# yohanshin/MultiviewHMR

Measured on AMD Instinct MI355X. Metric: Mvoxel*views/s (64^3 grid, 256ch, 4 views) fwd; max-abs vs ref, higher is better.
Workload: dtype f32

## Files before the change

### multiviewhmr_amd/csrc/brick_common.h

```cpp
#pragma once
#include <type_traits>
#include "device_common.h"

namespace mvhmr {

constexpr int kBZ = 32;
constexpr int kBX = 4;
constexpr int kMaxChunks = 5;
constexpr int brick_chunks_per_wave(int nt) { return nt >= 1024 ? kMaxChunks : 2 * kMaxChunks; }
constexpr int brick_view_slots(int v) { return v <= 2 ? 2 : v <= 4 ? 4 : 8; }

struct BrickTiles { int hx, hy, hz, share; bool split_x, split_y, split_z; };
__host__ __device__ inline BrickTiles brick_tiles(int nbx, int nby, int nbz)
{
    BrickTiles t;
    t.split_z = nbz >= 2;
    t.split_x = t.split_z ? nbx > nby : true;
    t.split_y = t.split_z ? !t.split_x : true;
    t.hx = t.split_x ? (nbx + 1) / 2 : nbx; t.hy = t.split_y ? (nby + 1) / 2 : nby; t.hz = t.split_z ? (nbz + 1) / 2 : nbz;
    t.share = t.hx * t.hy * t.hz;
    return t;
}

constexpr int kAbsentSlot = 64;
constexpr float kAbsentSample = -3.4028234663852886e38f;
constexpr int kZeroSlots = 128;
constexpr int kZeroBytes = kZeroSlots * 16;

__device__ __forceinline__ void lds_barrier()
{
    asm volatile("s_waitcnt lgkmcnt(0)\n\ts_barrier" ::: "memory");
}

__device__ __forceinline__ void bare_barrier()
{
    asm volatile("s_barrier" ::: "memory");
}
// ... 162 lines not shown
```

### multiviewhmr_amd/csrc/capi.hip

```cpp
#include "mvhmr_unproject.h"

#include <hip/hip_runtime.h>
#include <stdarg.h>
#include <stdio.h>

#include <mutex>
#include <unordered_map>

#include "device_common.h"
#include "kernels.h"

using namespace mvhmr;

namespace mvhmr {
unsigned long long dynamic_lds_cache_key(int device, const void *kernel)
{
    return (unsigned long long)reinterpret_cast<uintptr_t>(kernel) ^ ((unsigned long long)(unsigned)device << 56) ^ (unsigned long long)(device & 0xff);
}

hipError_t allow_dynamic_lds(const void *kernel, size_t bytes)
{
    static std::mutex mu;
    static std::unordered_map<unsigned long long, size_t> granted;
    int dev = 0;
    hipError_t e = hipGetDevice(&dev);
    if (e != hipSuccess) return e;
    const unsigned long long key = dynamic_lds_cache_key(dev, kernel);
    std::lock_guard<std::mutex> lock(mu);
    auto it = granted.find(key);
    if (it != granted.end() && it->second >= bytes) return hipSuccess;
    e = hipFuncSetAttribute(kernel, hipFuncAttributeMaxDynamicSharedMemorySize, (int)bytes);
    if (e == hipSuccess) granted[key] = bytes;
    return e;
}
}

namespace {

thread_local char g_err[512] = "";

int fail(int status, const char *fmt, ...)
{
    va_list ap;
    va_start(ap, fmt);
    vsnprintf(g_err, sizeof(g_err), fmt, ap);
    va_end(ap);
    return status;
}
// ... 88 lines not shown
bool gateable_layout(const mvhmr_unproject_desc *d, const Problem &p)
{
    return d->feat_layout == MVHMR_LAYOUT_BVCHW || (d->feat_layout == MVHMR_LAYOUT_QUAD && quad_to_channels_last_supported(p));
}
bool geometry_gated(const mvhmr_unproject_desc *d, const Problem &p)
{
    return d->variant == MVHMR_VARIANT_AUTO && gateable_layout(d, p) && brick_fwd_preferred(p);
}
bool geometry_gated_bwd(const mvhmr_unproject_desc *d, const Problem &p)
{
    return d->variant == MVHMR_VARIANT_AUTO && gateable_layout(d, p) && brick_bwd_supported(p);
}
constexpr size_t kGateBytes = 256;
size_t conv_bytes(const Problem &p) { const size_t a = featT_bytes(p), b = brick_workspace_bytes(p); return a > b ? a : b; }

int arm_gate(Problem &p, unsigned char *at, const float *proj, const Coords &coords, const GateGeom &g, hipStream_t s)
{
    int *count = reinterpret_cast<int *>(at);
    hipError_t e = hipMemsetAsync(count, 0, sizeof(int), s);
    if (e != hipSuccess) return fail(MVHMR_ERR_LAUNCH, "geometry gate clear: %s", hipGetErrorString(e));
    e = launch_brick_gate(proj, coords, count, g, p, s);
    if (e != hipSuccess) return fail(MVHMR_ERR_LAUNCH, "geometry gate: %s", hipGetErrorString(e));
    p.gate_count = count;
    p.gate_limit = brick_count(p, g) / 8;
    return MVHMR_OK;
}

int check_ws(void *ws, size_t have, size_t need)
{
    if (need == 0) return MVHMR_OK;
    if (!ws) return fail(MVHMR_ERR_WORKSPACE, "workspace is null but %zu bytes are required", need);
    if (have < need) return fail(MVHMR_ERR_WORKSPACE, "workspace has %zu bytes, %zu are required", have, need);
    if (reinterpret_cast<uintptr_t>(ws) % kAlign) return fail(MVHMR_ERR_WORKSPACE, "workspace must be %zu-byte aligned", kAlign);
    return MVHMR_OK;
}

Coords coords_from_tensor(const float *coords, const Problem &p)
{
    Coords c{};
// ... 416 lines not shown
}
int clear_gradient(void *acc, const Problem &p, size_t elem, hipStream_t s)
{
    return launched(hipMemsetAsync(acc, 0, (size_t)p.B * p.V * p.H * p.W * p.C4 * elem, s), "gradient clear");
}
int query_variant(const mvhmr_unproject_desc *desc, const VolumeSource &v, const float *proj, void *hip_stream)
{
    Problem p;
    if (check_desc(desc, &p) != MVHMR_OK) return -1;
    const int variant = pick_variant(desc, p);
    if (variant_conflict(desc, p, variant) != MVHMR_OK) return -1;
    if (desc->variant != MVHMR_VARIANT_AUTO || !brick_fwd_preferred(p)) return variant;
    Coords coords;
    if (!proj || make_coords(v, p, &coords) != MVHMR_OK) { fail(MVHMR_ERR_INVALID_ARGUMENT, v.cuboid ? "null pointer" : "proj / coords must be non-null"); return -1; }
    hipStream_t s = static_cast<hipStream_t>(hip_stream);
    int *count = nullptr, host = 0;
    if (hipMalloc(&count, sizeof(int)) != hipSuccess) { fail(MVHMR_ERR_LAUNCH, "query: allocation failed"); return -1; }
    hipError_t e = hipMemsetAsync(count, 0, sizeof(int), s);
    const GateGeom g = brick_fwd_gate_geom(p);
    if (e == hipSuccess) e = launch_brick_gate(proj, coords, count, g, p, s);
    if (e == hipSuccess) e = hipMemcpyAsync(&host, count, sizeof(int), hipMemcpyDeviceToHost, s);
    if (e == hipSuccess) e = hipStreamSynchronize(s);
    (void)hipFree(count);
    if (e != hipSuccess) { fail(MVHMR_ERR_LAUNCH, "query: %s", hipGetErrorString(e)); return -1; }
    return host <= brick_count(p, g) / 8 ? MVHMR_VARIANT_BRICK : MVHMR_VARIANT_GATHER;
}

int run_forward(const mvhmr_unproject_desc *desc, const VolumeSource &v, const void *features, const float *proj, const Views &views, void *out,
                void *workspace, size_t workspace_bytes, void *hip_stream, const SharedIndex *shared = nullptr, const LensArgs *lens = nullptr)
{
    Problem p0;
    Coords coords;
    int rc = open_call(desc, v, &p0, &coords);
    if (rc != MVHMR_OK) return rc;
    if (!features || !proj || !out) return fail(MVHMR_ERR_INVALID_ARGUMENT, "features / proj / out must be non-null");
    if ((rc = views_refused(desc, views)) != MVHMR_OK) return rc;
    if (shared && (rc = shared_refused(desc, *shared)) != MVHMR_OK) return rc;
    if (lens && (rc = lens_refused(desc, *lens)) != MVHMR_OK) return rc;
    if (lens) p0.lens = lens->lens;
    hipStream_t s = static_cast<hipStream_t>(hip_stream);
// ... 1097 lines not shown
```

### multiviewhmr_amd/csrc/device_common.h

```cpp
#pragma once
#include <hip/hip_runtime.h>
#include <hip/hip_fp16.h>
#include <stdint.h>
#include "gate.h"

namespace mvhmr {

__device__ __forceinline__ bool gated_off(const Gate &g)
{
    if (!g.count) return false;
    const bool brick = __builtin_nontemporal_load(g.count) <= g.limit;
    return brick != (g.wants_brick != 0);
}


__device__ __forceinline__ void cuboid_offset(const Coords &cs, int b, long long n, float &dx, float &dy, float &dz)
{
    const int k = (int)(n % cs.Z), j = (int)((n / cs.Z) % cs.Y), i = (int)(n / ((long long)cs.Y * cs.Z));
    const float *ce = cs.center + b * 3;
    const float gx = __fadd_rn(cs.px, __fmul_rn(cs.sx, (float)i));
    const float gy = __fadd_rn(cs.py, __fmul_rn(cs.sy, (float)j));
    const float gz = __fadd_rn(cs.pz, __fmul_rn(cs.sz, (float)k));
    dx = __fsub_rn(gx, ce[0]); dy = __fsub_rn(gy, ce[1]); dz = __fsub_rn(gz, ce[2]);
}

__device__ __forceinline__ void voxel_xyz(const Coords &cs, int b, long long N, long long n, float &x, float &y, float &z)
{
// ... 554 lines not shown
```

### multiviewhmr_amd/csrc/gate.h

```cpp
#pragma once

namespace mvhmr {

struct Gate {
    const int *count;
    int limit;
    int wants_brick;
};

struct Coords {
    const float *ptr;
    const float *rot;
    const float *center;
    float px, py, pz;
    float sx, sy, sz;
    int Y, Z;
};

}
```

### multiviewhmr_amd/csrc/kernels.h

```cpp
#pragma once
#include <hip/hip_runtime.h>
#include <stddef.h>
#include <stdint.h>
#include "gate.h"

namespace mvhmr {

struct Problem {
    int B, V, C, H, W;
    int X, Y, Z;
    long long N;
    int C4;
    int method;
    int feat_f16, out_f16;
    int out_bf16 = 0;
    int feat_log2e = 0;
    const int *gate_count = nullptr;
    int gate_limit = 0;
    const int *view_count = nullptr;
    const float *view_weights = nullptr;
    int masked = 0;
    int visible = 0;
    const float *confidence = nullptr;
    int conf = 0;
    float *conf_stream = nullptr;
    const int *feature_index = nullptr;
    int volumes = 0;
    const float *lens = nullptr;
};

inline Gate make_gate(const Problem &p, bool wants_brick) { return Gate{p.gate_count, p.gate_limit, wants_brick ? 1 : 0}; }


hipError_t allow_dynamic_lds(const void *kernel, size_t bytes);
unsigned long long dynamic_lds_cache_key(int device, const void *kernel);

hipError_t launch_to_channels_last(const void *src, void *dst, const Problem &p, hipStream_t s);
hipError_t launch_grad_to_planar(const float *srcT, void *dst, const Problem &p, hipStream_t s);
bool quad_to_channels_last_supported(const Problem &p);
hipError_t launch_quad_to_channels_last(const void *srcK, void *dst, const Problem &p, hipStream_t s);
hipError_t launch_grad_cast(const float *srcT, void *dst, const Problem &p, hipStream_t s);

hipError_t launch_fwd_gather(const void *featT, const float *proj, const Coords &coords, void *out,
                             const Problem &p, hipStream_t s);
hipError_t launch_bwd_gather(const void *grad_out, const void *featT, const float *proj, const Coords &coords,
                             float *gradT, const Problem &p, hipStream_t s);

// ... 25 lines not shown
hipError_t launch_bwd_plane(const void *featK, const void *grad_out, const float *proj, const Coords &coords, void *grad_features,
                            void *table, const Problem &p, hipStream_t s);

struct GateGeom {
    int bx, by, bz;
    int view_group;
    int column_major;
    int parity_rows;
    int cap_slots;
    int max_chunks;
};
GateGeom brick_fwd_gate_geom(const Problem &p);
GateGeom brick_bwd_gate_geom(const Problem &p);
hipError_t launch_brick_gate(const float *proj, const Coords &coords, int *count, const GateGeom &g, const Problem &p, hipStream_t s);
int brick_count(const Problem &p, const GateGeom &g);

hipError_t launch_bwd_brick(const void *featK, const void *grad_out, const float *proj, const Coords &coords, float *gradK,
                            const Problem &p, hipStream_t s);
hipError_t launch_quad_grad_to_planar(const float *gradK, void *dst, const Problem &p, hipStream_t s);

bool conv1x1_quad_supported(int Cin, int Cout, int H, int W);
bool conv1x1_planar_supported(int Cin, int Cout, int HW);
bool conv1x1_wgrad_supported(int Cin, int Cout, int HW);
hipError_t launch_conv1x1_wgrad(const float *gy, const float *x, float *dW, float *db, int BV, int Cin, int Cout, int HW, hipStream_t s);
size_t conv1x1_wgrad_det_workspace_bytes(int BV, int Cin, int Cout, int HW);
hipError_t launch_conv1x1_wgrad_det(const float *gy, const float *x, float *dW, float *db, void *ws, int BV, int Cin, int Cout, int HW, hipStream_t s);
constexpr int kConv1x1MaxMaps = 65535;
hipError_t launch_conv1x1_planar(const float *x, const float *w, const float *bias, float *dst, int BV, int Cin, int Cout, int HW, hipStream_t s);
hipError_t launch_conv1x1_quad(const float *x, const float *w, const float *bias, void *dst, int BV, int Cin, int Cout, int H, int W,
                               hipStream_t s);
// ... 81 lines not shown
```

### multiviewhmr_amd/csrc/unproject_brick_fwd.hip

```cpp
#include "brick_fwd_ws.h"

namespace mvhmr {

template <typename TF>
__global__ void __launch_bounds__(256)
k_to_quad_planar_t(const TF *__restrict__ src, float4 *__restrict__ dst, int C, int H, int W, float scale, Gate gate)
{
    if (gated_off(gate)) return;
    __shared__ float tile[4][32][33];
    const long long bv = blockIdx.z;
    const int q = blockIdx.y;
    const int tiles_x = (W + 31) >> 5;
    const int x0 = (blockIdx.x % tiles_x) << 5, y0 = (blockIdx.x / tiles_x) << 5;
    const int tx = threadIdx.x & 31, ty = threadIdx.x >> 5;
    const TF *s = src + (bv * C + q * 4) * (long long)H * W;
    const int nc = C - q * 4 < 4 ? C - q * 4 : 4;
#pragma unroll
    for (int c = 0; c < 4; ++c)
#pragma unroll
        for (int i = 0; i < 4; ++i) {
            const int y = y0 + ty + 8 * i, x = x0 + tx;
            if (y < H && x < W) tile[c][ty + 8 * i][tx] = c < nc ? to_f32<TF>(s[(long long)c * H * W + (long long)y * W + x]) * scale : 0.f;
        }
    __syncthreads();
// ... 148 lines not shown
    const int nt = brick_fwd_grouped(p) ? 1024 : fwd_threads(p.V);
    GateGeom g;
    g.bx = kBX * brick_fwd_nvox(p); g.by = nt / 128; g.bz = kBZ; g.column_major = 1;
    g.parity_rows = kFwdLay == 1 ? 1 : 0;
    g.view_group = brick_fwd_grouped(p) ? 4 : 0;
    g.cap_slots = fwd_cap2(fwd_lds_slots());
    g.max_chunks = brick_fwd_grouped(p) ? 4 * (nt / 64) : brick_chunks_per_wave(nt) * (nt / 64);
    return g;
}

int brick_count(const Problem &p, const GateGeom &g)
{
    return ((p.X + g.bx - 1) / g.bx) * ((p.Y + g.by - 1) / g.by) * ((p.Z + g.bz - 1) / g.bz) * p.B;
}

__global__ void __launch_bounds__(256)
k_brick_gate(const float *__restrict__ proj, const Coords coords, int *__restrict__ count, int V, int H, int W, int X,
             int Y, int Z, GateGeom g, int nbx, int nby, int nbz, int total)
{
    const int i = blockIdx.x * 256 + threadIdx.x;
    if (i >= total) return;
    const int bps = nbx * nby * nbz;
    const int b = i / bps, r = i % bps;
    const int kz = r % nbz, ky = (r / nbz) % nby, kx = r / (nbz * nby);
    const long long N = (long long)X * Y * Z;
    int used = 0, chunks_all = 0, max_stride = 0, used_max = 0, chunks_max = 0;
    for (int v = 0; v < V; ++v) {
        if (g.view_group && v % g.view_group == 0) { used = 0; chunks_all = 0; }
        const float *P = proj + ((long long)b * V + v) * 12;
        float xmin = 1e30f, xmax = -1e30f, ymin = 1e30f, ymax = -1e30f;
        bool front = true;
        for (int c = 0; c < 8; ++c) {
            int vx = kx * g.bx + ((c & 1) ? g.bx - 1 : 0), vy = ky * g.by + ((c & 2) ? g.by - 1 : 0), vz = kz * g.bz + ((c & 4) ? g.bz - 1 : 0);
            vx = vx < X ? vx : X - 1; vy = vy < Y ? vy : Y - 1; vz = vz < Z ? vz : Z - 1;
            float Xp[3];
            voxel_xyz(coords, b, N, ((long long)vx * Y + vy) * Z + vz, Xp[0], Xp[1], Xp[2]);
            const float a = P[0] * Xp[0] + P[1] * Xp[1] + P[2] * Xp[2] + P[3];
            const float bb = P[4] * Xp[0] + P[5] * Xp[1] + P[6] * Xp[2] + P[7];
            const float z = P[8] * Xp[0] + P[9] * Xp[1] + P[10] * Xp[2] + P[11];
            if (!(z > 0.f)) { front = false; continue; }
            const float ix = (a / z) / (float)H * (float)(W - 1), iy = (bb / z) / (float)W * (float)(H - 1);
            xmin = fminf(xmin, ix); xmax = fmaxf(xmax, ix); ymin = fminf(ymin, iy); ymax = fmaxf(ymax, iy);
        }
        if (!front || xmax < xmin) continue;
        const float x0 = fmaxf(floorf(xmin), -1.f), x1 = fminf(floorf(xmax), (float)(W - 1));
        const float y0 = fmaxf(floorf(ymin), -1.f), y1 = fminf(floorf(ymax), (float)(H - 1));
        if (x1 < x0 || y1 < y0) continue;
        const int bw = (int)(x1 - x0) + 2, bh = (int)(y1 - y0) + 2;
        int stride = (g.column_major ? bh : bw) | 1;
        const int lines = g.column_major ? bw : bh;
        if (g.parity_rows) {
            const int y0e = (int)y0 & ~1;
            stride = 2 * (((int)y1 + 3 - y0e) >> 1);
        }
        const int chunks = (stride * lines + 63) >> 6;
        used += chunks << 6;
        chunks_all += chunks;
        max_stride = stride > max_stride ? stride : max_stride;
        used_max = used > used_max ? used : used_max;
        chunks_max = chunks_all > chunks_max ? chunks_all : chunks_max;
    }
    const bool fits = used_max <= g.cap_slots && chunks_max <= g.max_chunks && max_stride + 2 <= kZeroSlots;
    if (!fits) atomicAdd(count, 1);
}

hipError_t launch_brick_gate(const float *proj, const Coords &coords, int *count, const GateGeom &g, const Problem &p, hipStream_t s)
{
    const int nbx = (p.X + g.bx - 1) / g.bx, nby = (p.Y + g.by - 1) / g.by, nbz = (p.Z + g.bz - 1) / g.bz, total = nbx * nby * nbz * p.B;
    hipLaunchKernelGGL(k_brick_gate, dim3((total + 255) / 256), dim3(256), 0, s, proj, coords, count, p.V, p.H, p.W, p.X, p.Y, p.Z, g,
                       nbx, nby, nbz, total);
    return hipGetLastError();
}

extern template hipError_t launch_fwd_method<AGG_SOFTMAX>(const void *, const float *, const Coords &, void *, const Problem &, int, hipStream_t);
extern template hipError_t launch_fwd_method<AGG_SUM>(const void *, const float *, const Coords &, void *, const Problem &, int, hipStream_t);
extern template hipError_t launch_fwd_method<AGG_MEAN>(const void *, const float *, const Coords &, void *, const Problem &, int, hipStream_t);
extern template hipError_t launch_fwd_method<AGG_MAX>(const void *, const float *, const Coords &, void *, const Problem &, int, hipStream_t);

template <int METHOD, int VT, typename TO>
__global__ void __launch_bounds__(256)
k_fwd_tail(const float4 *__restrict__ featK, const float *__restrict__ proj, const Coords coords, TO *__restrict__ out, int C, int H, int W, long long N,
           int nv, float unscale, Gate gate)
{
    if (gated_off(gate)) return;
// ... 58 lines not shown
```

### multiviewhmr_amd/csrc/unproject_gather.hip

```cpp
#include "device_common.h"
#include "det_scale.h"
#include "kernels.h"

namespace mvhmr {

constexpr int kTileVox = 32;
constexpr int kGroupQuads = 64;
constexpr int kGroupCh = 256;
constexpr unsigned kGatedTiles = 256;

struct alignas(16) TapRec {
    int o00, o01, o10, o11;
    float w00, w01, w10, w11;
};

__device__ __forceinline__ void build_records(TapRec *recs, const float *__restrict__ proj,
                                              const Coords &coords, int b, int V, long long n0,
                                              long long N, int H, int W, int C4)
{
    for (int idx = threadIdx.x; idx < kTileVox * V; idx += blockDim.x) {
        const int v = idx / kTileVox, j = idx % kTileVox;
        long long n = n0 + j;
        n = n < N ? n : N - 1;
        float X0, X1, X2;
// ... 20 lines not shown
    __builtin_nontemporal_store(__builtin_bit_cast(unsigned short, (bf16_t)v), reinterpret_cast<unsigned short *>(p));
}

struct UTap { int o00, o01, o10, o11; float w00, w01, w10, w11; };
__device__ __forceinline__ UTap uniform_rec(const TapRec &r)
{
    UTap u;
    u.o00 = uniform(r.o00); u.o01 = uniform(r.o01); u.o10 = uniform(r.o10); u.o11 = uniform(r.o11);
    u.w00 = uniform(r.w00); u.w01 = uniform(r.w01); u.w10 = uniform(r.w10); u.w11 = uniform(r.w11);
    return u;
}

template <typename TF, typename TO, int METHOD, int VT, bool MASK = false>
__global__ void __launch_bounds__(256)
k_fwd_gather(const TF *__restrict__ featT, const float *__restrict__ proj, const Coords coords,
             TO *__restrict__ out, int Vrt, int C, int C4, int H, int W, long long N, int tstride, Gate gate, const int *__restrict__ nvs = nullptr)
{
    if (gated_off(gate)) return;
    const int V = VT > 0 ? VT : Vrt;
    const int nvb = MASK ? nvs[blockIdx.y] : V;
    extern __shared__ __align__(16) unsigned char smem[];
    TapRec *recs = reinterpret_cast<TapRec *>(smem);
    f32x4 *tile = reinterpret_cast<f32x4 *>(smem + sizeof(TapRec) * kTileVox * V);
    const int tid = threadIdx.x, lane = tid & 63, wave = tid >> 6;
    const int b = blockIdx.y, cg = blockIdx.z;
    for (long long n0 = (long long)blockIdx.x * kTileVox; n0 < N; n0 += (long long)gridDim.x * kTileVox) {
    const long long mapsz = (long long)H * W * C4;
    const int Q = C4 >> 2;

    build_records(recs, proj, coords, b, V, n0, N, H, W, C4);
    __syncthreads();

    int q = cg * kGroupQuads + lane;
    const bool q_active = q < Q;
    q = q_active ? q : Q - 1;
    const TF *fb = featT + (long long)b * V * mapsz + q * 4;

    for (int jj = 0; jj < kTileVox / 4; ++jj) {
        const int j = wave * (kTileVox / 4) + jj;
        f32x4 o;
        if constexpr (VT > 0) {
// ... 545 lines not shown
                float sv[4], dsv[4];
                sample4(u, v, sv);
                const float wv = wb[v];
#pragma unroll
                for (int i = 0; i < 4; ++i) dsv[i] = ra[i].grad(g[i], sv[i], wv);
                scatter4(u, v, dsv);
            }
        }
    }
    __syncthreads();
    }
}

template <typename T, bool VEC>
__global__ void __launch_bounds__(256)
k_to_channels_last(const T *__restrict__ src, T *__restrict__ dst, int C, int C4, int HW, Gate gate)
{
    if (gated_off(gate)) return;
    __shared__ T t[64][65];
    const long long bv = blockIdx.z;
    const int p0 = blockIdx.x * 64, c0 = blockIdx.y * 64;
    if constexpr (VEC) {
        struct alignas(sizeof(T) * 4) V4 { T x, y, z, w; };
        const int l16 = threadIdx.x & 15, g = threadIdx.x >> 4;
        for (int r = g; r < 64; r += 16) {
            const int c = c0 + r, p = p0 + 4 * l16;
            V4 v = {from_f32<T>(0.f), from_f32<T>(0.f), from_f32<T>(0.f), from_f32<T>(0.f)};
            if (c < C && p < HW) v = *reinterpret_cast<const V4 *>(src + (bv * C + c) * HW + p);
            t[r][4 * l16] = v.x; t[r][4 * l16 + 1] = v.y; t[r][4 * l16 + 2] = v.z; t[r][4 * l16 + 3] = v.w;
        }
        __syncthreads();
        for (int r = g; r < 64; r += 16) {
            const int p = p0 + r, c = c0 + 4 * l16;
            if (p < HW && c < C4) {
                const V4 v = {t[4 * l16][r], t[4 * l16 + 1][r], t[4 * l16 + 2][r], t[4 * l16 + 3][r]};
                *reinterpret_cast<V4 *>(dst + (bv * HW + p) * C4 + c) = v;
            }
        }
    } else {
        const int lane = threadIdx.x & 63, w = threadIdx.x >> 6;
        for (int r = w; r < 64; r += 4) {
            const int c = c0 + r, p = p0 + lane;
            t[r][lane] = (c < C && p < HW) ? src[(bv * C + c) * HW + p] : from_f32<T>(0.f);
        }
        __syncthreads();
        for (int r = w; r < 64; r += 4) {
            const int p = p0 + r, c = c0 + lane;
            if (p < HW && c < C4) dst[(bv * HW + p) * C4 + c] = t[lane][r];
        }
    }
}

template <typename T>
__global__ void __launch_bounds__(256)
k_quad_to_channels_last(const float4 *__restrict__ src, T *__restrict__ dst, int C, int H, int W, int band_log2, Gate gate)
{
    if (gated_off(gate)) return;
    extern __shared__ float4 qtile[];
    const int nq = C >> 2, ldq = nq | 1, band = 1 << band_log2;
    const long long bv = blockIdx.y;
    const int bands = (H + band - 1) >> band_log2;
    const int x = blockIdx.x / bands, y0 = (blockIdx.x % bands) << band_log2;
    const int rows = H - y0 < band ? H - y0 : band;
    const long long HW = (long long)H * W;
    const float4 *sp = src + bv * nq * HW + (long long)x * H + y0;
    for (int i = threadIdx.x; i < band * nq; i += 256) {
        const int q = i >> band_log2, r = i & (band - 1);
        if (r < rows) qtile[r * ldq + q] = sp[(long long)q * HW + r];
    }
    __syncthreads();
    for (int i = threadIdx.x; i < rows * nq; i += 256) {
        const int r = i / nq, q = i - r * nq;
        const float4 v = qtile[r * ldq + q];
        Vec4<T>::store(dst + ((bv * HW + (long long)(y0 + r) * W + x) * C + 4 * q), f32x4{{v.x, v.y, v.z, v.w}});
    }
}

template <typename T>
__global__ void __launch_bounds__(256)
k_grad_to_planar(const float *__restrict__ srcT, T *__restrict__ dst, int C, int C4, int HW, Gate gate)
{
    if (gated_off(gate)) return;
    __shared__ float t[64][65];
    const int lane = threadIdx.x & 63, w = threadIdx.x >> 6;
    const long long bv = blockIdx.z;
    const int p0 = blockIdx.x * 64, c0 = blockIdx.y * 64;
    for (int r = w; r < 64; r += 4) {
        const int p = p0 + r, c = c0 + lane;
        t[r][lane] = (p < HW && c < C4) ? srcT[(bv * HW + p) * C4 + c] : 0.f;
// ... 31 lines not shown
    for (int r = 0; r < 3; ++r) {
        const float acc = __fmaf_rn(R[r * 3 + 2], dz, __fmaf_rn(R[r * 3 + 1], dy, __fmul_rn(R[r * 3 + 0], dx)));
        o[r] = __fadd_rn(acc, ce[r]);
    }
}

template <typename TF, typename TO, int METHOD>
static hipError_t fwd_dispatch_v(const TF *featT, const float *proj, const Coords &coords, TO *out, const Problem &p,
                                 hipStream_t s)
{
    const int Q = p.C4 / 4;
    int tstride = (Q < kGroupQuads ? Q : kGroupQuads) + 1;
    tstride |= 1;
    const size_t lds = sizeof(TapRec) * kTileVox * (size_t)p.V + sizeof(f32x4) * kTileVox * (size_t)tstride;
    const unsigned tiles = (unsigned)((p.N + kTileVox - 1) / kTileVox);
    const dim3 grid(p.gate_count && tiles > kGatedTiles ? kGatedTiles : tiles, (unsigned)p.B, (unsigned)((Q + kGroupQuads - 1) / kGroupQuads));
    auto go = [&](auto kern) -> hipError_t {
        hipError_t e = allow_dynamic_lds(reinterpret_cast<const void *>(kern), lds);
        if (e != hipSuccess) return e;
        hipLaunchKernelGGL(kern, grid, dim3(256), lds, s, featT, proj, coords, out, p.V, p.C, p.C4, p.H, p.W, p.N, tstride, make_gate(p, false),
                           p.view_count);
        return hipGetLastError();
    };
    auto go_weighted = [&](auto kern) -> hipError_t {
        hipError_t e = allow_dynamic_lds(reinterpret_cast<const void *>(kern), lds);
        if (e != hipSuccess) return e;
        hipLaunchKernelGGL(kern, grid, dim3(256), lds, s, featT, proj, coords, out, p.V, p.C, p.C4, p.H, p.W, p.N, tstride, make_gate(p, false),
                           p.view_count, p.view_weights);
        return hipGetLastError();
    };
    if (p.view_weights) {
        if constexpr (METHOD == AGG_MAX) return hipErrorNotSupported;
        else switch (p.V) {
        case 2: return go_weighted(k_fwd_gather_weighted<TF, TO, METHOD, 2>);
        case 4: return go_weighted(k_fwd_gather_weighted<TF, TO, METHOD, 4>);
        case 8: return go_weighted(k_fwd_gather_weighted<TF, TO, METHOD, 8>);
        default: return go_weighted(k_fwd_gather_weighted<TF, TO, METHOD, 0>);
        }
    }
    if (p.view_count) {
        switch (p.V) {
// ... 30 lines not shown
    if (p.confidence) return launch_fwd_gather_conf(featT, proj, coords, out, p, s);
    if (p.visible) return launch_fwd_gather_seen(featT, proj, coords, out, p, s);
    if (p.out_bf16) return p.feat_f16 ? hipErrorNotSupported : fwd_dispatch_m((const float *)featT, proj, coords, (bf16_t *)out, p, s);
    if (!p.feat_f16 && !p.out_f16) return fwd_dispatch_m((const float *)featT, proj, coords, (float *)out, p, s);
    if (p.feat_f16 && p.out_f16) return fwd_dispatch_m((const __half *)featT, proj, coords, (__half *)out, p, s);
    if (p.feat_f16 && !p.out_f16) return fwd_dispatch_m((const __half *)featT, proj, coords, (float *)out, p, s);
    return hipErrorNotSupported;
}

template <typename TF, typename TO, int METHOD>
static hipError_t bwd_dispatch_v(const TO *go_, const TF *featT, const float *proj, const Coords &coords, float *gradT,
                                 const Problem &p, hipStream_t s)
{
    const size_t lds = sizeof(TapRec) * kTileVox * (size_t)p.V + sizeof(float) * kGroupCh * (kTileVox + 1);
    const unsigned tiles = (unsigned)((p.N + kTileVox - 1) / kTileVox);
    const dim3 grid(p.gate_count && tiles > kGatedTiles ? kGatedTiles : tiles, (unsigned)p.B, (unsigned)((p.C + kGroupCh - 1) / kGroupCh));
    auto go = [&](auto kern) -> hipError_t {
        hipError_t e = allow_dynamic_lds(reinterpret_cast<const void *>(kern), lds);
        if (e != hipSuccess) return e;
        hipLaunchKernelGGL(kern, grid, dim3(256), lds, s, go_, featT, proj, coords, gradT, p.V, p.C, p.C4, p.H, p.W, p.N, make_gate(p, false),
                           p.view_count);
        return hipGetLastError();
    };
    auto go_weighted = [&](auto kern) -> hipError_t {
        hipError_t e = allow_dynamic_lds(reinterpret_cast<const void *>(kern), lds);
        if (e != hipSuccess) return e;
        hipLaunchKernelGGL(kern, grid, dim3(256), lds, s, go_, featT, proj, coords, gradT, (const int *)nullptr, p.V, p.C, p.C4, p.H, p.W, p.N,
                           make_gate(p, false), p.view_count, p.view_weights);
        return hipGetLastError();
    };
    if (p.view_weights) {
// ... 112 lines not shown
hipError_t launch_bwd_gather_det(const void *grad_out, const void *featT, const float *proj, const Coords &coords, unsigned long long *gradI,
                                 const int *kexp, const Problem &p, hipStream_t s)
{
    if (p.confidence) return launch_bwd_gather_conf_det(grad_out, featT, proj, coords, gradI, kexp, p, s);
    if (p.visible) return launch_bwd_gather_seen_det(grad_out, featT, proj, coords, gradI, kexp, p, s);
    if (p.out_bf16) return p.feat_f16 ? hipErrorNotSupported : bwd_det_dispatch_m((const bf16_t *)grad_out, (const float *)featT, proj, coords, gradI, kexp, p, s);
    if (!p.feat_f16 && !p.out_f16) return bwd_det_dispatch_m((const float *)grad_out, (const float *)featT, proj, coords, gradI, kexp, p, s);
    if (p.feat_f16 && p.out_f16) return bwd_det_dispatch_m((const __half *)grad_out, (const __half *)featT, proj, coords, gradI, kexp, p, s);
    if (p.feat_f16 && !p.out_f16) return bwd_det_dispatch_m((const float *)grad_out, (const __half *)featT, proj, coords, gradI, kexp, p, s);
    return hipErrorNotSupported;
}

hipError_t launch_to_channels_last(const void *src, void *dst, const Problem &p, hipStream_t s)
{
    const int HW = p.H * p.W;
    const dim3 grid((HW + 63) / 64, (p.C4 + 63) / 64, (unsigned)(p.B * p.V));
    const bool vec = HW % 4 == 0 && p.C4 % 4 == 0 && (reinterpret_cast<size_t>(src) | reinterpret_cast<size_t>(dst)) % 16 == 0;
    const Gate gate = make_gate(p, false);
    if (p.feat_f16) {
        if (vec) hipLaunchKernelGGL((k_to_channels_last<__half, true>), grid, dim3(256), 0, s, (const __half *)src, (__half *)dst, p.C, p.C4, HW, gate);
        else hipLaunchKernelGGL((k_to_channels_last<__half, false>), grid, dim3(256), 0, s, (const __half *)src, (__half *)dst, p.C, p.C4, HW, gate);
    } else {
        if (vec) hipLaunchKernelGGL((k_to_channels_last<float, true>), grid, dim3(256), 0, s, (const float *)src, (float *)dst, p.C, p.C4, HW, gate);
        else hipLaunchKernelGGL((k_to_channels_last<float, false>), grid, dim3(256), 0, s, (const float *)src, (float *)dst, p.C, p.C4, HW, gate);
    }
    return hipGetLastError();
}

static int quad_band_log2(const Problem &p)
{
    for (int b = 5; b >= 2; --b)
        if (((size_t)((p.C / 4) | 1) * sizeof(float4) << b) <= 64 * 1024) return b;
    return -1;
}

bool quad_to_channels_last_supported(const Problem &p)
{
    return p.C % 4 == 0 && quad_band_log2(p) >= 0 && (long long)p.B * p.V <= 65535;
}

hipError_t launch_quad_to_channels_last(const void *srcK, void *dst, const Problem &p, hipStream_t s)
{
    if (!quad_to_channels_last_supported(p)) return hipErrorNotSupported;
    const int b = quad_band_log2(p);
    const size_t lds = (size_t)((p.C / 4) | 1) * sizeof(float4) << b;
    const dim3 grid((unsigned)(p.W * ((p.H + (1 << b) - 1) >> b)), (unsigned)(p.B * p.V));
    if (p.feat_f16) hipLaunchKernelGGL(k_quad_to_channels_last<__half>, grid, dim3(256), lds, s, (const float4 *)srcK, (__half *)dst, p.C, p.H, p.W, b, make_gate(p, false));
    else hipLaunchKernelGGL(k_quad_to_channels_last<float>, grid, dim3(256), lds, s, (const float4 *)srcK, (float *)dst, p.C, p.H, p.W, b, make_gate(p, false));
    return hipGetLastError();
}

hipError_t launch_grad_to_planar(const float *srcT, void *dst, const Problem &p, hipStream_t s)
{
    const int HW = p.H * p.W;
    const dim3 grid((HW + 63) / 64, (p.C4 + 63) / 64, (unsigned)(p.B * p.V));
    if (p.feat_f16) hipLaunchKernelGGL(k_grad_to_planar<__half>, grid, dim3(256), 0, s, srcT, (__half *)dst, p.C, p.C4, HW, make_gate(p, false));
    else hipLaunchKernelGGL(k_grad_to_planar<float>, grid, dim3(256), 0, s, srcT, (float *)dst, p.C, p.C4, HW, make_gate(p, false));
    return hipGetLastError();
}

hipError_t launch_grad_cast(const float *srcT, void *dst, const Problem &p, hipStream_t s)
{
    const long long n = (long long)p.B * p.V * p.H * p.W * p.C4;
// ... 146 lines not shown
```

Measured before the change: 9554.

## Parallelize geometry gate per-wave, drop memset, and persist gated kernel grids

The brick gate kernel now assigns one wave per brick, with 8 lanes covering corners and 8 view slots, and reduces across lanes with shuffles. Each block writes a partial count, which removes the atomic and the separate hipMemsetAsync launch. Gated-off fallback kernels (gather, channels-last transposes) now launch a persistent grid capped at CUs×8 and walk the logical blocks, so fewer dead blocks are launched when the gate turns them off. The cost is that gated_off now reads up to 64 partial counts per block instead of one int, and persistent loops need extra barriers.

```diff
diff --git a/multiviewhmr_amd/csrc/brick_common.h b/multiviewhmr_amd/csrc/brick_common.h
--- a/multiviewhmr_amd/csrc/brick_common.h
+++ b/multiviewhmr_amd/csrc/brick_common.h
@@ -21,6 +21,8 @@
     t.share = t.hx * t.hy * t.hz;
     return t;
 }
+
+constexpr int kGatedBlocksPerCU = 8;
 
 constexpr int kAbsentSlot = 64;
 constexpr float kAbsentSample = -3.4028234663852886e38f;
diff --git a/multiviewhmr_amd/csrc/capi.hip b/multiviewhmr_amd/csrc/capi.hip
--- a/multiviewhmr_amd/csrc/capi.hip
+++ b/multiviewhmr_amd/csrc/capi.hip
@@ -7,6 +7,7 @@
 #include <mutex>
 #include <unordered_map>
 
+#include "brick_common.h"
 #include "device_common.h"
 #include "kernels.h"
 
@@ -32,6 +33,22 @@
     e = hipFuncSetAttribute(kernel, hipFuncAttributeMaxDynamicSharedMemorySize, (int)bytes);
     if (e == hipSuccess) granted[key] = bytes;
     return e;
+}
+
+unsigned gated_block_cap()
+{
+    static std::mutex mu;
+    static std::unordered_map<int, unsigned> cus;
+    int dev = 0;
+    if (hipGetDevice(&dev) != hipSuccess) return 0;
+    std::lock_guard<std::mutex> lock(mu);
+    auto it = cus.find(dev);
+    if (it == cus.end()) {
+        int n = 0;
+        if (hipDeviceGetAttribute(&n, hipDeviceAttributeMultiprocessorCount, dev) != hipSuccess || n < 1) return 0;
+        it = cus.emplace(dev, (unsigned)n).first;
+    }
+    return it->second * kGatedBlocksPerCU;
 }
 }
 
@@ -150,15 +167,16 @@
 constexpr size_t kGateBytes = 256;
 size_t conv_bytes(const Problem &p) { const size_t a = featT_bytes(p), b = brick_workspace_bytes(p); return a > b ? a : b; }
 
+static_assert(kGateParts * sizeof(int) == kGateBytes, "one int per block of k_brick_gate");
+
 int arm_gate(Problem &p, unsigned char *at, const float *proj, const Coords &coords, const GateGeom &g, hipStream_t s)
 {
     int *count = reinterpret_cast<int *>(at);
-    hipError_t e = hipMemsetAsync(count, 0, sizeof(int), s);
-    if (e != hipSuccess) return fail(MVHMR_ERR_LAUNCH, "geometry gate clear: %s", hipGetErrorString(e));
-    e = launch_brick_gate(proj, coords, count, g, p, s);
+    const hipError_t e = launch_brick_gate(proj, coords, count, g, p, s);
     if (e != hipSuccess) return fail(MVHMR_ERR_LAUNCH, "geometry gate: %s", hipGetErrorString(e));
     p.gate_count = count;
     p.gate_limit = brick_count(p, g) / 8;
+    p.gate_parts = gate_parts(brick_count(p, g));
     return MVHMR_OK;
 }
 
@@ -605,16 +623,18 @@
     Coords coords;
     if (!proj || make_coords(v, p, &coords) != MVHMR_OK) { fail(MVHMR_ERR_INVALID_ARGUMENT, v.cuboid ? "null pointer" : "proj / coords must be non-null"); return -1; }
     hipStream_t s = static_cast<hipStream_t>(hip_stream);
-    int *count = nullptr, host = 0;
-    if (hipMalloc(&count, sizeof(int)) != hipSuccess) { fail(MVHMR_ERR_LAUNCH, "query: allocation failed"); return -1; }
-    hipError_t e = hipMemsetAsync(count, 0, sizeof(int), s);
+    int *count = nullptr, host[kGateParts];
+    if (hipMalloc(&count, kGateBytes) != hipSuccess) { fail(MVHMR_ERR_LAUNCH, "query: allocation failed"); return -1; }
     const GateGeom g = brick_fwd_gate_geom(p);
-    if (e == hipSuccess) e = launch_brick_gate(proj, coords, count, g, p, s);
-    if (e == hipSuccess) e = hipMemcpyAsync(&host, count, sizeof(int), hipMemcpyDeviceToHost, s);
+    const int parts = gate_parts(brick_count(p, g));
+    hipError_t e = launch_brick_gate(proj, coords, count, g, p, s);
+    if (e == hipSuccess) e = hipMemcpyAsync(host, count, parts * sizeof(int), hipMemcpyDeviceToHost, s);
     if (e == hipSuccess) e = hipStreamSynchronize(s);
     (void)hipFree(count);
     if (e != hipSuccess) { fail(MVHMR_ERR_LAUNCH, "query: %s", hipGetErrorString(e)); return -1; }
-    return host <= brick_count(p, g) / 8 ? MVHMR_VARIANT_BRICK : MVHMR_VARIANT_GATHER;
+    int overflowing = 0;
+    for (int i = 0; i < parts; ++i) overflowing += host[i];
+    return overflowing <= brick_count(p, g) / 8 ? MVHMR_VARIANT_BRICK : MVHMR_VARIANT_GATHER;
 }
 
 int run_forward(const mvhmr_unproject_desc *desc, const VolumeSource &v, const void *features, const float *proj, const Views &views, void *out,
diff --git a/multiviewhmr_amd/csrc/device_common.h b/multiviewhmr_amd/csrc/device_common.h
--- a/multiviewhmr_amd/csrc/device_common.h
+++ b/multiviewhmr_amd/csrc/device_common.h
@@ -9,8 +9,28 @@
 __device__ __forceinline__ bool gated_off(const Gate &g)
 {
     if (!g.count) return false;
-    const bool brick = __builtin_nontemporal_load(g.count) <= g.limit;
+    const int4 *c = reinterpret_cast<const int4 *>(g.count);
+    int4 v[kGateParts / 4];
+#pragma unroll
+    for (int i = 0; i < kGateParts / 4; ++i) v[i] = c[i];
+    int sum = 0;
+#pragma unroll
+    for (int i = 0; i < kGateParts / 4; ++i) {
+        sum += i == 0 || 4 * i < g.parts ? v[i].x : 0;
+        sum += 4 * i + 1 < g.parts ? v[i].y : 0;
+        sum += 4 * i + 2 < g.parts ? v[i].z : 0;
+        sum += 4 * i + 3 < g.parts ? v[i].w : 0;
+    }
+    const bool brick = sum <= g.limit;
     return brick != (g.wants_brick != 0);
+}
+
+__device__ __forceinline__ unsigned walk_end(const Walk &w) { return w.nx ? w.nx * w.ny * w.nz : blockIdx.x + 1; }
+__device__ __forceinline__ uint3 walk_at(const Walk &w, unsigned blk)
+{
+    if (!w.nx) return make_uint3(blockIdx.x, blockIdx.y, blockIdx.z);
+    const unsigned row = blk / w.nx;
+    return make_uint3(blk - row * w.nx, row % w.ny, row / w.ny);
 }
 
 
diff --git a/multiviewhmr_amd/csrc/gate.h b/multiviewhmr_amd/csrc/gate.h
--- a/multiviewhmr_amd/csrc/gate.h
+++ b/multiviewhmr_amd/csrc/gate.h
@@ -1,11 +1,18 @@
 #pragma once
 
 namespace mvhmr {
+
+constexpr int kGateParts = 64;
 
 struct Gate {
     const int *count;
     int limit;
     int wants_brick;
+    int parts;
+};
+
+struct Walk {
+    unsigned nx, ny, nz;
 };
 
 struct Coords {
diff --git a/multiviewhmr_amd/csrc/kernels.h b/multiviewhmr_amd/csrc/kernels.h
--- a/multiviewhmr_amd/csrc/kernels.h
+++ b/multiviewhmr_amd/csrc/kernels.h
@@ -17,6 +17,7 @@
     int feat_log2e = 0;
     const int *gate_count = nullptr;
     int gate_limit = 0;
+    int gate_parts = 0;
     const int *view_count = nullptr;
     const float *view_weights = nullptr;
     int masked = 0;
@@ -29,8 +30,17 @@
     const float *lens = nullptr;
 };
 
-inline Gate make_gate(const Problem &p, bool wants_brick) { return Gate{p.gate_count, p.gate_limit, wants_brick ? 1 : 0}; }
+inline Gate make_gate(const Problem &p, bool wants_brick) { return Gate{p.gate_count, p.gate_limit, wants_brick ? 1 : 0, p.gate_parts}; }
 
+unsigned gated_block_cap();
+inline dim3 walk_grid(const Problem &p, const dim3 &logical, Walk *w)
+{
+    const unsigned long long n = (unsigned long long)logical.x * logical.y * logical.z;
+    const unsigned cap = p.gate_count ? gated_block_cap() : 0;
+    if (!cap || n <= cap || n > 0x7fffffffull) { *w = Walk{0, 0, 0}; return logical; }
+    *w = Walk{logical.x, logical.y, logical.z};
+    return dim3(cap);
+}
 
 hipError_t allow_dynamic_lds(const void *kernel, size_t bytes);
 unsigned long long dynamic_lds_cache_key(int device, const void *kernel);
@@ -86,6 +96,7 @@
 GateGeom brick_bwd_gate_geom(const Problem &p);
 hipError_t launch_brick_gate(const float *proj, const Coords &coords, int *count, const GateGeom &g, const Problem &p, hipStream_t s);
 int brick_count(const Problem &p, const GateGeom &g);
+int gate_parts(int bricks);
 
 hipError_t launch_bwd_brick(const void *featK, const void *grad_out, const float *proj, const Coords &coords, float *gradK,
                             const Problem &p, hipStream_t s);
diff --git a/multiviewhmr_amd/csrc/unproject_brick_fwd.hip b/multiviewhmr_amd/csrc/unproject_brick_fwd.hip
--- a/multiviewhmr_amd/csrc/unproject_brick_fwd.hip
+++ b/multiviewhmr_amd/csrc/unproject_brick_fwd.hip
@@ -186,60 +186,99 @@
     return ((p.X + g.bx - 1) / g.bx) * ((p.Y + g.by - 1) / g.by) * ((p.Z + g.bz - 1) / g.bz) * p.B;
 }
 
-__global__ void __launch_bounds__(256)
+struct GateWindow { int chunks, stride; };
+__device__ __forceinline__ GateWindow gate_window(float xmin, float xmax, float ymin, float ymax, bool front, const GateGeom &g, int H, int W)
+{
+    GateWindow w;
+    w.chunks = w.stride = 0;
+    if (!front || xmax < xmin) return w;
+    const float x0 = fmaxf(floorf(xmin), -1.f), x1 = fminf(floorf(xmax), (float)(W - 1));
+    const float y0 = fmaxf(floorf(ymin), -1.f), y1 = fminf(floorf(ymax), (float)(H - 1));
+    if (x1 < x0 || y1 < y0) return w;
+    const int bw = (int)(x1 - x0) + 2, bh = (int)(y1 - y0) + 2;
+    int stride = (g.column_major ? bh : bw) | 1;
+    const int lines = g.column_major ? bw : bh;
+    if (g.parity_rows) {
+        const int y0e = (int)y0 & ~1;
+        stride = 2 * (((int)y1 + 3 - y0e) >> 1);
+    }
+    w.chunks = (stride * lines + 63) >> 6;
+    w.stride = stride;
+    return w;
+}
+
+constexpr int kGateWaves = 16;
+__global__ void __launch_bounds__(kGateWaves * 64)
 k_brick_gate(const float *__restrict__ proj, const Coords coords, int *__restrict__ count, int V, int H, int W, int X,
              int Y, int Z, GateGeom g, int nbx, int nby, int nbz, int total)
 {
-    const int i = blockIdx.x * 256 + threadIdx.x;
-    if (i >= total) return;
+    __shared__ int wave_count[kGateWaves];
+    const int lane = threadIdx.x & 63, wave = threadIdx.x >> 6;
+    const int c = lane & 7, slot = lane >> 3;
     const int bps = nbx * nby * nbz;
-    const int b = i / bps, r = i % bps;
-    const int kz = r % nbz, ky = (r / nbz) % nby, kx = r / (nbz * nby);
     const long long N = (long long)X * Y * Z;
-    int used = 0, chunks_all = 0, max_stride = 0, used_max = 0, chunks_max = 0;
-    for (int v = 0; v < V; ++v) {
-        if (g.view_group && v % g.view_group == 0) { used = 0; chunks_all = 0; }
-        const float *P = proj + ((long long)b * V + v) * 12;
-        float xmin = 1e30f, xmax = -1e30f, ymin = 1e30f, ymax = -1e30f;
-        bool front = true;
-        for (int c = 0; c < 8; ++c) {
-            int vx = kx * g.bx + ((c & 1) ? g.bx - 1 : 0), vy = ky * g.by + ((c & 2) ? g.by - 1 : 0), vz = kz * g.bz + ((c & 4) ? g.bz - 1 : 0);
-            vx = vx < X ? vx : X - 1; vy = vy < Y ? vy : Y - 1; vz = vz < Z ? vz : Z - 1;
-            float Xp[3];
-            voxel_xyz(coords, b, N, ((long long)vx * Y + vy) * Z + vz, Xp[0], Xp[1], Xp[2]);
-            const float a = P[0] * Xp[0] + P[1] * Xp[1] + P[2] * Xp[2] + P[3];
-            const float bb = P[4] * Xp[0] + P[5] * Xp[1] + P[6] * Xp[2] + P[7];
-            const float z = P[8] * Xp[0] + P[9] * Xp[1] + P[10] * Xp[2] + P[11];
-            if (!(z > 0.f)) { front = false; continue; }
-            const float ix = (a / z) / (float)H * (float)(W - 1), iy = (bb / z) / (float)W * (float)(H - 1);
-            xmin = fminf(xmin, ix); xmax = fmaxf(xmax, ix); ymin = fminf(ymin, iy); ymax = fmaxf(ymax, iy);
+    int overflowing = 0;
+    for (int i = blockIdx.x * kGateWaves + wave; i < total; i += gridDim.x * kGateWaves) {
+        const int b = i / bps, r = i % bps;
+        const int kz = r % nbz, ky = (r / nbz) % nby, kx = r / (nbz * nby);
+        int vx = kx * g.bx + ((c & 1) ? g.bx - 1 : 0), vy = ky * g.by + ((c & 2) ? g.by - 1 : 0), vz = kz * g.bz + ((c & 4) ? g.bz - 1 : 0);
+        vx = vx < X ? vx : X - 1; vy = vy < Y ? vy : Y - 1; vz = vz < Z ? vz : Z - 1;
+        float Xp[3];
+        voxel_xyz(coords, b, N, ((long long)vx * Y + vy) * Z + vz, Xp[0], Xp[1], Xp[2]);
+        int used = 0, chunks_all = 0, max_stride = 0, used_max = 0, chunks_max = 0;
+        for (int v0 = 0; v0 < V; v0 += 8) {
+            const int v = v0 + slot;
+            float xmin = 1e30f, xmax = -1e30f, ymin = 1e30f, ymax = -1e30f;
+            int front = 1;
+            if (v < V) {
+                const float *P = proj + ((long long)b * V + v) * 12;
+                const float a = P[0] * Xp[0] + P[1] * Xp[1] + P[2] * Xp[2] + P[3];
+                const float bb = P[4] * Xp[0] + P[5] * Xp[1] + P[6] * Xp[2] + P[7];
+                const float z = P[8] * Xp[0] + P[9] * Xp[1] + P[10] * Xp[2] + P[11];
+                if (!(z > 0.f)) {
+                    front = 0;
+                } else {
+                    const float ix = (a / z) / (float)H * (float)(W - 1), iy = (bb / z) / (float)W * (float)(H - 1);
+                    xmin = fminf(xmin, ix); xmax = fmaxf(xmax, ix); ymin = fminf(ymin, iy); ymax = fmaxf(ymax, iy);
+                }
+            }
+#pragma unroll
+            for (int m = 1; m < 8; m <<= 1) {
+                xmin = fminf(xmin, __shfl_xor(xmin, m)); xmax = fmaxf(xmax, __shfl_xor(xmax, m));
+                ymin = fminf(ymin, __shfl_xor(ymin, m)); ymax = fmaxf(ymax, __shfl_xor(ymax, m));
+                front &= __shfl_xor(front, m);
+            }
+            const GateWindow w = gate_window(xmin, xmax, ymin, ymax, front != 0, g, H, W);
+            const int nv = V - v0 < 8 ? V - v0 : 8;
+            for (int k = 0; k < nv; ++k) {
+                if (g.view_group && (v0 + k) % g.view_group == 0) { used = 0; chunks_all = 0; }
+                const int chunks = __shfl(w.chunks, k * 8), stride = __shfl(w.stride, k * 8);
+                used += chunks << 6;
+                chunks_all += chunks;
+                max_stride = stride > max_stride ? stride : max_stride;
+                used_max = used > used_max ? used : used_max;
+                chunks_max = chunks_all > chunks_max ? chunks_all : chunks_max;
+            }
         }
-        if (!front || xmax < xmin) continue;
-        const float x0 = fmaxf(floorf(xmin), -1.f), x1 = fminf(floorf(xmax), (float)(W - 1));
-        const float y0 = fmaxf(floorf(ymin), -1.f), y1 = fminf(floorf(ymax), (float)(H - 1));
-        if (x1 < x0 || y1 < y0) continue;
-        const int bw = (int)(x1 - x0) + 2, bh = (int)(y1 - y0) + 2;
-        int stride = (g.column_major ? bh : bw) | 1;
-        const int lines = g.column_major ? bw : bh;
-        if (g.parity_rows) {
-            const int y0e = (int)y0 & ~1;
-            stride = 2 * (((int)y1 + 3 - y0e) >> 1);
-        }
-        const int chunks = (stride * lines + 63) >> 6;
-        used += chunks << 6;
-        chunks_all += chunks;
-        max_stride = stride > max_stride ? stride : max_stride;
-        used_max = used > used_max ? used : used_max;
-        chunks_max = chunks_all > chunks_max ? chunks_all : chunks_max;
-    }
-    const bool fits = used_max <= g.cap_slots && chunks_max <= g.max_chunks && max_stride + 2 <= kZeroSlots;
-    if (!fits) atomicAdd(count, 1);
-}
+        const bool fits = used_max <= g.cap_slots && chunks_max <= g.max_chunks && max_stride + 2 <= kZeroSlots;
+        overflowing += fits ? 0 : 1;
+    }
+    if (lane == 0) wave_count[wave] = overflowing;
+    __syncthreads();
+    if (threadIdx.x == 0) {
+        int sum = 0;
+#pragma unroll
+        for (int w = 0; w < kGateWaves; ++w) sum += wave_count[w];
+        count[blockIdx.x] = sum;
+    }
+}
+
+int gate_parts(int bricks) { const int blocks = (bricks + kGateWaves - 1) / kGateWaves; return blocks < kGateParts ? blocks : kGateParts; }
 
 hipError_t launch_brick_gate(const float *proj, const Coords &coords, int *count, const GateGeom &g, const Problem &p, hipStream_t s)
 {
     const int nbx = (p.X + g.bx - 1) / g.bx, nby = (p.Y + g.by - 1) / g.by, nbz = (p.Z + g.bz - 1) / g.bz, total = nbx * nby * nbz * p.B;
-    hipLaunchKernelGGL(k_brick_gate, dim3((total + 255) / 256), dim3(256), 0, s, proj, coords, count, p.V, p.H, p.W, p.X, p.Y, p.Z, g,
+    hipLaunchKernelGGL(k_brick_gate, dim3(gate_parts(total)), dim3(kGateWaves * 64), 0, s, proj, coords, count, p.V, p.H, p.W, p.X, p.Y, p.Z, g,
                        nbx, nby, nbz, total);
     return hipGetLastError();
 }
diff --git a/multiviewhmr_amd/csrc/unproject_gather.hip b/multiviewhmr_amd/csrc/unproject_gather.hip
--- a/multiviewhmr_amd/csrc/unproject_gather.hip
+++ b/multiviewhmr_amd/csrc/unproject_gather.hip
@@ -1,3 +1,4 @@
+#include "brick_common.h"
 #include "device_common.h"
 #include "det_scale.h"
 #include "kernels.h"
@@ -7,7 +8,11 @@
 constexpr int kTileVox = 32;
 constexpr int kGroupQuads = 64;
 constexpr int kGroupCh = 256;
-constexpr unsigned kGatedTiles = 256;
+static unsigned gated_tiles(const Problem &p, unsigned tiles)
+{
+    const unsigned cus = p.gate_count ? gated_block_cap() / kGatedBlocksPerCU : 0;
+    return cus && tiles > cus ? cus : tiles;
+}
 
 struct alignas(16) TapRec {
     int o00, o01, o10, o11;
@@ -58,17 +63,20 @@
 template <typename TF, typename TO, int METHOD, int VT, bool MASK = false>
 __global__ void __launch_bounds__(256)
 k_fwd_gather(const TF *__restrict__ featT, const float *__restrict__ proj, const Coords coords,
-             TO *__restrict__ out, int Vrt, int C, int C4, int H, int W, long long N, int tstride, Gate gate, const int *__restrict__ nvs = nullptr)
+             TO *__restrict__ out, int Vrt, int C, int C4, int H, int W, long long N, int tstride, Gate gate, Walk walk,
+             const int *__restrict__ nvs = nullptr)
 {
     if (gated_off(gate)) return;
     const int V = VT > 0 ? VT : Vrt;
-    const int nvb = MASK ? nvs[blockIdx.y] : V;
     extern __shared__ __align__(16) unsigned char smem[];
     TapRec *recs = reinterpret_cast<TapRec *>(smem);
     f32x4 *tile = reinterpret_cast<f32x4 *>(smem + sizeof(TapRec) * kTileVox * V);
     const int tid = threadIdx.x, lane = tid & 63, wave = tid >> 6;
-    const int b = blockIdx.y, cg = blockIdx.z;
-    for (long long n0 = (long long)blockIdx.x * kTileVox; n0 < N; n0 += (long long)gridDim.x * kTileVox) {
+    for (unsigned blk = blockIdx.x, end = walk_end(walk); blk < end; blk += gridDim.x) {
+    const uint3 at = walk_at(walk, blk);
+    const int b = at.y, cg = at.z;
+    const int nvb = MASK ? nvs[b] : V;
+    const long long n0 = (long long)at.x * kTileVox;
     const long long mapsz = (long long)H * W * C4;
     const int Q = C4 >> 2;
 
@@ -644,12 +652,14 @@
 
 template <typename T, bool VEC>
 __global__ void __launch_bounds__(256)
-k_to_channels_last(const T *__restrict__ src, T *__restrict__ dst, int C, int C4, int HW, Gate gate)
+k_to_channels_last(const T *__restrict__ src, T *__restrict__ dst, int C, int C4, int HW, Gate gate, Walk walk)
 {
     if (gated_off(gate)) return;
     __shared__ T t[64][65];
-    const long long bv = blockIdx.z;
-    const int p0 = blockIdx.x * 64, c0 = blockIdx.y * 64;
+    for (unsigned blk = blockIdx.x, end = walk_end(walk); blk < end; blk += gridDim.x) {
+    const uint3 at = walk_at(walk, blk);
+    const long long bv = at.z;
+    const int p0 = at.x * 64, c0 = at.y * 64;
     if constexpr (VEC) {
         struct alignas(sizeof(T) * 4) V4 { T x, y, z, w; };
         const int l16 = threadIdx.x & 15, g = threadIdx.x >> 4;
@@ -679,18 +689,22 @@
             if (p < HW && c < C4) dst[(bv * HW + p) * C4 + c] = t[lane][r];
         }
     }
+    __syncthreads();
+    }
 }
 
 template <typename T>
 __global__ void __launch_bounds__(256)
-k_quad_to_channels_last(const float4 *__restrict__ src, T *__restrict__ dst, int C, int H, int W, int band_log2, Gate gate)
+k_quad_to_channels_last(const float4 *__restrict__ src, T *__restrict__ dst, int C, int H, int W, int band_log2, Gate gate, Walk walk)
 {
     if (gated_off(gate)) return;
     extern __shared__ float4 qtile[];
     const int nq = C >> 2, ldq = nq | 1, band = 1 << band_log2;
-    const long long bv = blockIdx.y;
     const int bands = (H + band - 1) >> band_log2;
-    const int x = blockIdx.x / bands, y0 = (blockIdx.x % bands) << band_log2;
+    for (unsigned blk = blockIdx.x, end = walk_end(walk); blk < end; blk += gridDim.x) {
+    const uint3 at = walk_at(walk, blk);
+    const long long bv = at.y;
+    const int x = at.x / bands, y0 = (at.x % bands) << band_log2;
     const int rows = H - y0 < band ? H - y0 : band;
     const long long HW = (long long)H * W;
     const float4 *sp = src + bv * nq * HW + (long long)x * H + y0;
@@ -703,6 +717,8 @@
         const int r = i / nq, q = i - r * nq;
         const float4 v = qtile[r * ldq + q];
         Vec4<T>::store(dst + ((bv * HW + (long long)(y0 + r) * W + x) * C + 4 * q), f32x4{{v.x, v.y, v.z, v.w}});
+    }
+    __syncthreads();
     }
 }
 
@@ -764,17 +780,20 @@
     tstride |= 1;
     const size_t lds = sizeof(TapRec) * kTileVox * (size_t)p.V + sizeof(f32x4) * kTileVox * (size_t)tstride;
     const unsigned tiles = (unsigned)((p.N + kTileVox - 1) / kTileVox);
-    const dim3 grid(p.gate_count && tiles > kGatedTiles ? kGatedTiles : tiles, (unsigned)p.B, (unsigned)((Q + kGroupQuads - 1) / kGroupQuads));
+    const unsigned groups = (unsigned)((Q + kGroupQuads - 1) / kGroupQuads);
     auto go = [&](auto kern) -> hipError_t {
         hipError_t e = allow_dynamic_lds(reinterpret_cast<const void *>(kern), lds);
         if (e != hipSuccess) return e;
-        hipLaunchKernelGGL(kern, grid, dim3(256), lds, s, featT, proj, coords, out, p.V, p.C, p.C4, p.H, p.W, p.N, tstride, make_gate(p, false),
+        Walk walk;
+        const dim3 grid = walk_grid(p, dim3(tiles, (unsigned)p.B, groups), &walk);
+        hipLaunchKernelGGL(kern, grid, dim3(256), lds, s, featT, proj, coords, out, p.V, p.C, p.C4, p.H, p.W, p.N, tstride, make_gate(p, false), walk,
                            p.view_count);
         return hipGetLastError();
     };
     auto go_weighted = [&](auto kern) -> hipError_t {
         hipError_t e = allow_dynamic_lds(reinterpret_cast<const void *>(kern), lds);
         if (e != hipSuccess) return e;
+        const dim3 grid(gated_tiles(p, tiles), (unsigned)p.B, groups);
         hipLaunchKernelGGL(kern, grid, dim3(256), lds, s, featT, proj, coords, out, p.V, p.C, p.C4, p.H, p.W, p.N, tstride, make_gate(p, false),
                            p.view_count, p.view_weights);
         return hipGetLastError();
@@ -835,7 +854,7 @@
 {
     const size_t lds = sizeof(TapRec) * kTileVox * (size_t)p.V + sizeof(float) * kGroupCh * (kTileVox + 1);
     const unsigned tiles = (unsigned)((p.N + kTileVox - 1) / kTileVox);
-    const dim3 grid(p.gate_count && tiles > kGatedTiles ? kGatedTiles : tiles, (unsigned)p.B, (unsigned)((p.C + kGroupCh - 1) / kGroupCh));
+    const dim3 grid(gated_tiles(p, tiles), (unsigned)p.B, (unsigned)((p.C + kGroupCh - 1) / kGroupCh));
     auto go = [&](auto kern) -> hipError_t {
         hipError_t e = allow_dynamic_lds(reinterpret_cast<const void *>(kern), lds);
         if (e != hipSuccess) return e;
@@ -978,15 +997,16 @@
 hipError_t launch_to_channels_last(const void *src, void *dst, const Problem &p, hipStream_t s)
 {
     const int HW = p.H * p.W;
-    const dim3 grid((HW + 63) / 64, (p.C4 + 63) / 64, (unsigned)(p.B * p.V));
+    Walk walk;
+    const dim3 grid = walk_grid(p, dim3((HW + 63) / 64, (p.C4 + 63) / 64, (unsigned)(p.B * p.V)), &walk);
     const bool vec = HW % 4 == 0 && p.C4 % 4 == 0 && (reinterpret_cast<size_t>(src) | reinterpret_cast<size_t>(dst)) % 16 == 0;
     const Gate gate = make_gate(p, false);
     if (p.feat_f16) {
-        if (vec) hipLaunchKernelGGL((k_to_channels_last<__half, true>), grid, dim3(256), 0, s, (const __half *)src, (__half *)dst, p.C, p.C4, HW, gate);
-        else hipLaunchKernelGGL((k_to_channels_last<__half, false>), grid, dim3(256), 0, s, (const __half *)src, (__half *)dst, p.C, p.C4, HW, gate);
+        if (vec) hipLaunchKernelGGL((k_to_channels_last<__half, true>), grid, dim3(256), 0, s, (const __half *)src, (__half *)dst, p.C, p.C4, HW, gate, walk);
+        else hipLaunchKernelGGL((k_to_channels_last<__half, false>), grid, dim3(256), 0, s, (const __half *)src, (__half *)dst, p.C, p.C4, HW, gate, walk);
     } else {
-        if (vec) hipLaunchKernelGGL((k_to_channels_last<float, true>), grid, dim3(256), 0, s, (const float *)src, (float *)dst, p.C, p.C4, HW, gate);
-        else hipLaunchKernelGGL((k_to_channels_last<float, false>), grid, dim3(256), 0, s, (const float *)src, (float *)dst, p.C, p.C4, HW, gate);
+        if (vec) hipLaunchKernelGGL((k_to_channels_last<float, true>), grid, dim3(256), 0, s, (const float *)src, (float *)dst, p.C, p.C4, HW, gate, walk);
+        else hipLaunchKernelGGL((k_to_channels_last<float, false>), grid, dim3(256), 0, s, (const float *)src, (float *)dst, p.C, p.C4, HW, gate, walk);
     }
     return hipGetLastError();
 }
@@ -1008,9 +1028,10 @@
     if (!quad_to_channels_last_supported(p)) return hipErrorNotSupported;
     const int b = quad_band_log2(p);
     const size_t lds = (size_t)((p.C / 4) | 1) * sizeof(float4) << b;
-    const dim3 grid((unsigned)(p.W * ((p.H + (1 << b) - 1) >> b)), (unsigned)(p.B * p.V));
-    if (p.feat_f16) hipLaunchKernelGGL(k_quad_to_channels_last<__half>, grid, dim3(256), lds, s, (const float4 *)srcK, (__half *)dst, p.C, p.H, p.W, b, make_gate(p, false));
-    else hipLaunchKernelGGL(k_quad_to_channels_last<float>, grid, dim3(256), lds, s, (const float4 *)srcK, (float *)dst, p.C, p.H, p.W, b, make_gate(p, false));
+    Walk walk;
+    const dim3 grid = walk_grid(p, dim3((unsigned)(p.W * ((p.H + (1 << b) - 1) >> b)), (unsigned)(p.B * p.V)), &walk);
+    if (p.feat_f16) hipLaunchKernelGGL(k_quad_to_channels_last<__half>, grid, dim3(256), lds, s, (const float4 *)srcK, (__half *)dst, p.C, p.H, p.W, b, make_gate(p, false), walk);
+    else hipLaunchKernelGGL(k_quad_to_channels_last<float>, grid, dim3(256), lds, s, (const float4 *)srcK, (float *)dst, p.C, p.H, p.W, b, make_gate(p, false), walk);
     return hipGetLastError();
 }
 
```

After: 9568, median of 2. No clear change (+0.1%).
